# limanling/clip-event

Hardware: AMD Instinct MI355X
Metric: image-text pairs/sec/GPU, ViT-B/32 224px x 77-tok, global-batch contrastive (higher is better)
Workload: dtype bf16; 1 GPU; ViT-B/32 224px x 77-tok, bf16 operands, per-GPU batch 256, K=1, InfoNCE only, full train step (fwd+bwd+clip_grad_norm+Adam), random-init weights; global_batch=256, parallelism=dp1, captions=SOT + U[8,75] random ids + EOT, zero-padded to 77 (SURVEY 8(d) c2), text_rows=live tokens SOT..EOT only: 54.8% of B*77 rows (identical results, see DESIGN.md), fresh_captions_every_step=True, alignment=False, cu_hog=0, nt_pgrid=256, full=False

## Files before the change

### clip_event_amd/csrc/embed.hip

```cpp
#include <limits.h>

#include "common.hpp"
#include "../../include/clip_event_hip.h"

namespace {

__device__ __forceinline__ void im2col_group(const float* __restrict__ img, bf16_t* __restrict__ out_row, int b, int gy,
                                             int gx, int cg, int R, int ps) {
    if (ps % 8 == 0 && R % 4 == 0) {
        const int col = cg * 8;
        u32x4 pk = {0u, 0u, 0u, 0u};
        if (col < 3 * ps * ps) {
            const int c = col / (ps * ps), py = (col / ps) % ps, px = col % ps;
            const float* src = img + (((long)b * 3 + c) * R + gy * ps + py) * R + gx * ps + px;
            const f32x4 lo = __builtin_nontemporal_load(reinterpret_cast<const f32x4*>(src));
            const f32x4 hi = __builtin_nontemporal_load(reinterpret_cast<const f32x4*>(src + 4));
            pk = u32x4{pack_bf2(lo[0], lo[1]), pack_bf2(lo[2], lo[3]), pack_bf2(hi[0], hi[1]), pack_bf2(hi[2], hi[3])};
        }
        *reinterpret_cast<u32x4*>(out_row + cg * 8) = pk;
        return;
    }
    float v[8];
#pragma unroll
    for (int e = 0; e < 8; ++e) {
// ... 365 lines not shown
    }
    if (lane == 0) rows[r] = (int)(r * Ltok + arg);
}

__global__ void copy_rows_kernel(const char* __restrict__ src, long src_stride, const int* __restrict__ src_rows,
                                 char* __restrict__ dst, long dst_stride, const int* __restrict__ dst_rows, int n,
                                 int chunks) {
    const long total = (long)n * chunks;
    for (long idx = blockIdx.x * (long)blockDim.x + threadIdx.x; idx < total; idx += (long)gridDim.x * blockDim.x) {
        const int i = (int)(idx / chunks), c = (int)(idx - (long)i * chunks);
        const long sr = src_rows ? src_rows[i] : i, dr = dst_rows ? dst_rows[i] : i;
        *reinterpret_cast<u32x4*>(dst + dr * dst_stride + c * 16L) =
            *reinterpret_cast<const u32x4*>(src + sr * src_stride + c * 16L);
    }
}

__global__ void scatter_rows_zero_kernel(const char* __restrict__ src, long src_stride, char* __restrict__ dst, long dst_stride,
                                         const int* __restrict__ dst_rows, int n, int M, int chunks) {
    const long total = (long)M * chunks;
    for (long idx = blockIdx.x * (long)blockDim.x + threadIdx.x; idx < total; idx += (long)gridDim.x * blockDim.x) {
        const int r = (int)(idx / chunks), c = (int)(idx - (long)r * chunks);
        int lo = 0, hi = n - 1;
        while (lo < hi) {
            const int mid = (lo + hi) >> 1;
            if (dst_rows[mid] < r) lo = mid + 1;
            else hi = mid;
        }
        u32x4 v = {0u, 0u, 0u, 0u};
        if (dst_rows[lo] == r) v = *reinterpret_cast<const u32x4*>(src + (long)lo * src_stride + c * 16L);
        *reinterpret_cast<u32x4*>(dst + (long)r * dst_stride + c * 16L) = v;
    }
}

int grid_for(long threads, int block = 256, int cap = 8192) {
    long g = (threads + block - 1) / block;
    return (int)(g > cap ? cap : (g < 1 ? 1 : g));
}

}

extern "C" int ce_im2col(const float* image, void* patches, int B, int resolution, int patch, int k_padded,
                         void* stream) {
    CE_CHECK_ARG(B > 0 && patch > 0 && resolution % patch == 0, "ce_im2col: resolution %d not a multiple of patch %d", resolution, patch);
    CE_CHECK_ARG(k_padded % 8 == 0 && k_padded >= 3 * patch * patch, "ce_im2col: k_padded must be a multiple of 8 >= 3*patch^2");
    const int grid = resolution / patch;
    const long threads = (long)B * grid * grid * (k_padded / 8);
    hipLaunchKernelGGL(im2col_kernel, dim3(grid_for(threads)), dim3(256), 0, (hipStream_t)stream, image,
                       (bf16_t*)patches, B, resolution, patch, grid, k_padded);
    CE_LAUNCH_CHECK();
    return 0;
}

extern "C" int ce_vision_assemble(const float* patch_out, const float* cls, const float* pos, float* x0, int B,
                                  int tokens, int D, void* stream) {
    CE_CHECK_ARG(B > 0 && tokens > 1 && D % 4 == 0, "ce_vision_assemble: bad shape");
    hipLaunchKernelGGL(vision_assemble_kernel, dim3(grid_for((long)B * tokens * (D / 4))), dim3(256), 0,
                       (hipStream_t)stream, patch_out, cls, pos, x0, B, tokens, D);
    CE_LAUNCH_CHECK();
    return 0;
}

extern "C" int ce_vision_assemble_bwd(const float* dx0, void* dpatch, int B, int tokens, int D, void* stream) {
    CE_CHECK_ARG(B > 0 && tokens > 1 && D % 4 == 0, "ce_vision_assemble_bwd: bad shape");
    hipLaunchKernelGGL(vision_assemble_bwd_kernel, dim3(grid_for((long)B * (tokens - 1) * (D / 4))), dim3(256), 0,
                       (hipStream_t)stream, dx0, (bf16_t*)dpatch, B, tokens, D);
    CE_LAUNCH_CHECK();
// ... 149 lines not shown
    return 0;
}

extern "C" int ce_scatter_rows_zero(const void* src, long src_stride_bytes, void* dst, long dst_stride_bytes,
                                    const int* dst_rows, int n, int M, int row_bytes, void* stream) {
    CE_CHECK_ARG(n > 0 && M >= n && row_bytes > 0 && row_bytes % 16 == 0 && src_stride_bytes % 16 == 0 && dst_stride_bytes % 16 == 0 &&
                 dst_rows, "ce_scatter_rows_zero: rows must be multiples of 16 bytes, 0 < n <= M");
    const int chunks = row_bytes / 16;
    hipLaunchKernelGGL(scatter_rows_zero_kernel, dim3(grid_for((long)M * chunks)), dim3(256), 0, (hipStream_t)stream,
                       (const char*)src, src_stride_bytes, (char*)dst, dst_stride_bytes, dst_rows, n, M, chunks);
    CE_LAUNCH_CHECK();
    return 0;
}

extern "C" int ce_eot_rows(const int64_t* ids, int* rows, long n, int tokens, void* stream) {
    CE_CHECK_ARG(n > 0 && tokens > 0, "ce_eot_rows: bad shape");
    hipLaunchKernelGGL(eot_rows_kernel, dim3((unsigned)((n + 3) / 4)), dim3(256), 0, (hipStream_t)stream,
                       (const long*)ids, rows, n, tokens);
    CE_LAUNCH_CHECK();
    return 0;
}

extern "C" int ce_copy_rows(const void* src, long src_stride_bytes, const int* src_rows, void* dst,
                            long dst_stride_bytes, const int* dst_rows, int n, int row_bytes, void* stream) {
    CE_CHECK_ARG(n > 0 && row_bytes > 0 && row_bytes % 16 == 0 && src_stride_bytes % 16 == 0 && dst_stride_bytes % 16 == 0,
                 "ce_copy_rows: rows must be multiples of 16 bytes");
    const int chunks = row_bytes / 16;
    hipLaunchKernelGGL(copy_rows_kernel, dim3(grid_for((long)n * chunks)), dim3(256), 0, (hipStream_t)stream,
                       (const char*)src, src_stride_bytes, src_rows, (char*)dst, dst_stride_bytes, dst_rows, n, chunks);
    CE_LAUNCH_CHECK();
    return 0;
}

namespace {
__global__ __launch_bounds__(256) void cu_hog_kernel(unsigned long long ticks, unsigned int* sink, int mode) {
    extern __shared__ unsigned int hog_lds[];
    const unsigned long long t0 = __builtin_amdgcn_s_memrealtime(), c0 = __builtin_amdgcn_s_memtime();
    unsigned int n = 0;
    while (__builtin_amdgcn_s_memrealtime() - t0 < ticks) {
        if (mode == 0) __builtin_amdgcn_s_sleep(32);
        else if (mode == 1) __builtin_amdgcn_s_sleep(127);
        ++n;
    }
    hog_lds[threadIdx.x & 255] = n;
    if (sink && threadIdx.x == 0 && blockIdx.x == 0) {
        const unsigned long long c1 = __builtin_amdgcn_s_memtime(), r1 = __builtin_amdgcn_s_memrealtime();
        reinterpret_cast<unsigned long long*>(sink)[0] = c1 - c0;
        reinterpret_cast<unsigned long long*>(sink)[1] = r1 - t0;
        sink[4] = hog_lds[(threadIdx.x + 1) & 255];
    }
}
}

static unsigned int* g_hog_sink = nullptr;
extern "C" double ce_cu_hog_clock_mhz(void) {
    if (!g_hog_sink) return 0.0;
    unsigned long long h[2] = {0, 0};
    hipDeviceSynchronize();
    hipMemcpy(h, g_hog_sink, sizeof(h), hipMemcpyDeviceToHost);
    return h[1] ? (double)h[0] / (double)h[1] * 100.0 : 0.0;
}

extern "C" int ce_cu_hog(int blocks, float microseconds, void* stream) {
    CE_CHECK_ARG(blocks > 0 && blocks <= 256 && microseconds > 0.f && microseconds <= 1.0e6f, "ce_cu_hog: blocks 1..256, time up to 1 s");
    static bool attr = false;
    if (!attr) {
// ... 16 lines not shown
```

### clip_event_amd/csrc/gemm.hip

```cpp
#include <stdlib.h>

#include <map>
#include <mutex>
#include <type_traits>

#include "common.hpp"
#include "nt_plan.hpp"
#include "tn_plan.hpp"
#include "../../include/clip_event_hip.h"

#ifndef CE_DIAG_TN3
#define CE_DIAG_TN3 0
#endif

namespace {

constexpr int NT_BM = 128, NT_BN = 128, NT_BK = 64;
constexpr int NT_STAGE_BYTES = (NT_BM + NT_BN) * NT_BK * 2;
constexpr int NT_LDS_BYTES = 2 * NT_STAGE_BYTES;

#include "gemm_common.hpp"

template <int EPI>
__global__ __launch_bounds__(256, 2) void gemm_nt_kernel(NTArgs p) {
// ... 1247 lines not shown
#pragma unroll
    for (int nt = 0; nt < 2; ++nt)
#pragma unroll
        for (int kt = 0; kt < 2; ++kt) {
            const int k = ek + kt * 32;
            if (k >= p.Kk) continue;
#pragma unroll
            for (int r = 0; r < 16; ++r) {
                const int n = en + nt * 32 + (r & 3) + 8 * (r >> 2);
                if (n < p.Nn) atomicAdd(p.out + (long)n * p.ldo + k, acc[nt][kt][r]);
            }
        }
}

constexpr int T2_TILE_BYTES = TN_BM * 256;
constexpr int T2_STAGE_BYTES = 2 * T2_TILE_BYTES;
constexpr int T2_LDS_BYTES = 2 * T2_STAGE_BYTES;

__device__ __forceinline__ bf16x8 tr_frag2(const char* p) {
    typedef __attribute__((address_space(3))) s16x4 lds_s16x4;
    s16x4 lo = __builtin_amdgcn_ds_read_tr16_b64_v4i16((lds_s16x4*)(p));
    s16x4 hi = __builtin_amdgcn_ds_read_tr16_b64_v4i16((lds_s16x4*)(p + 4 * 256));
    typedef __attribute__((ext_vector_type(8))) short s16x8;
    s16x8 v = {lo[0], lo[1], lo[2], lo[3], hi[0], hi[1], hi[2], hi[3]};
    return __builtin_bit_cast(bf16x8, v);
}

struct TNGroup {
    int count, splits, m_per_split, M, depth;
    int overwrite = 0;
    int tile_end[CE_TN_MAX_GROUP];
    TNArgs prob[CE_TN_MAX_GROUP];
};

__global__ __launch_bounds__(256, 2) void gemm_tn2_kernel(TNGroup grp) {
    extern __shared__ __attribute__((aligned(16))) char smem[];
    const int tid = threadIdx.x;
    const int lane = tid & 63;
    const int wave = __builtin_amdgcn_readfirstlane(tid >> 6);
    const int wn = wave >> 1, wk = wave & 1;

    const int m_tiles = (grp.M + TN_BM - 1) / TN_BM;
    const int mps = grp.m_per_split / TN_BM;
    const int s_r = lane >> 4;
    const int s_chunk = (lane & 15) ^ (s_r << 2);
    const int g = lane >> 4, li = lane & 15;
    const int t_row = 8 * (g >> 1) + (li >> 2);
    const int t_sw = (li >> 2) << 2;
    const int t_cb = 2 * (g & 1) + ((li & 3) >> 1);
    int offP[2], offQ[2];
#pragma unroll
    for (int t = 0; t < 2; ++t) {
        offP[t] = t_row * 256 + (((wn * 8 + t * 4 + t_cb) ^ t_sw) << 4) + (li & 1) * 8;
        offQ[t] = T2_TILE_BYTES + t_row * 256 + (((wk * 8 + t * 4 + t_cb) ^ t_sw) << 4) + (li & 1) * 8;
    }

    {
        const int lb = xcd_remap(blockIdx.x, gridDim.x);
        int tile = lb / grp.splits;
        const int mt0 = (lb - tile * grp.splits) * mps;
        const int mt1 = min(m_tiles, mt0 + mps);
        if (mt0 >= mt1) return;
        int pi = 0;
        while (pi + 1 < grp.count && tile >= grp.tile_end[pi]) ++pi;
        if (pi > 0) tile -= grp.tile_end[pi - 1];
        const TNArgs& p = grp.prob[pi];
// ... 624 lines not shown

extern "C" int ce_gemm_tn_grouped_ex(int count, const void* const* P, const long* ldp, const void* const* Q,
                                     const long* ldq, int M, const int* Nn, const int* Kk, float* const* out,
                                     const long* ldo, int splits, int overwrite, void* stream) {
    CE_CHECK_ARG(count >= 1 && count <= CE_TN_MAX_GROUP && M > 0, "ce_gemm_tn_grouped: 1..%d problems, M > 0", CE_TN_MAX_GROUP);
    hipStream_t s = (hipStream_t)stream;
    TNGroup g;
    g.count = count;
    g.M = M;
    double flops = 0.0, bytes = 0.0;
    long ldmax = 0;
    for (int i = 0; i < count; ++i) {
        CE_CHECK_ARG(Nn[i] > 0 && Kk[i] > 0, "ce_gemm_tn: empty problem");
        CE_CHECK_ARG(Nn[i] % 8 == 0 && Kk[i] % 8 == 0 && ldp[i] % 8 == 0 && ldq[i] % 8 == 0,
                     "ce_gemm_tn: Nn,Kk,ldp,ldq must be multiples of 8");
        CE_CHECK_ARG(ldp[i] >= Nn[i] && ldq[i] >= Kk[i] && ldo[i] >= Kk[i], "ce_gemm_tn: leading dimension smaller than the row");
        TNArgs& a = g.prob[i];
        a.P = (const bf16_t*)P[i]; a.ldp = ldp[i]; a.Q = (const bf16_t*)Q[i]; a.ldq = ldq[i];
        a.out = out[i]; a.ldo = ldo[i]; a.M = M; a.Nn = Nn[i]; a.Kk = Kk[i];
        flops += 2.0 * M * Nn[i] * Kk[i];
        bytes += 2.0 * ((double)M * Nn[i] + (double)M * Kk[i]) + 8.0 * Nn[i] * Kk[i];
        if (ldp[i] > ldmax) ldmax = ldp[i];
        if (ldq[i] > ldmax) ldmax = ldq[i];
    }
    CE_CHECK_ARG((long)M * ldmax * 2 < (1L << 32), "ce_gemm_tn: operand exceeds 4 GiB");

    const TNPlan p = tn_plan(M, count, Nn, Kk, splits, overwrite != 0, tn_process_knobs());
    g.splits = p.splits; g.m_per_split = p.m_per_split; g.depth = p.depth; g.overwrite = p.kernel_overwrites;
    for (int i = 0; i < CE_TN_MAX_GROUP; ++i) g.tile_end[i] = p.tile_end[i];
    for (int i = 0; i < count; ++i) {
        TNArgs& a = g.prob[i];
        a.tiles_n = p.tiles_n[i]; a.tiles_k = p.tiles_k[i]; a.splits = p.splits; a.m_per_split = p.m_per_split;
    }
    if (p.zero_fill_first)
        for (int i = 0; i < count; ++i)
            if (hipMemset2DAsync(out[i], (size_t)ldo[i] * 4, 0, (size_t)Kk[i] * 4, (size_t)Nn[i], s) != hipSuccess) {
                ce_set_error("ce_gemm_tn_grouped: zero-fill of output %d failed", i);
                return -5;
            }

    constexpr auto key = [](int form, int rows) { return 64 * form + rows; };
#define CE_TN_CASE(FORM, ROWS, ...)                                                      \
    case key(FORM, ROWS): {                                                              \
        CeProfScope prof(p.prof_class, flops, bytes, s);                                 \
        launch_kernel<__VA_ARGS__>(p.workgroups, p.block, p.lds_bytes, g, s);            \
    } break
    switch (key(p.form, p.rows)) {
        case key(TN_V1, 64):
            for (int i = 0; i < count; ++i) {
                const TNArgs& a = g.prob[i];
                CeProfScope prof(p.prof_class, 2.0 * M * a.Nn * a.Kk, 0.0, s);
                launch_kernel<gemm_tn_kernel>(a.tiles_n * a.tiles_k * a.splits, p.block, p.lds_bytes, a, s);
            }
            break;
        CE_TN_CASE(TN_V2, 64, gemm_tn2_kernel);
        CE_TN_CASE(TN_V3, 32, gemm_tn3_kernel<32, 4>);
        CE_TN_CASE(TN_V3, 48, gemm_tn3_kernel<48, 3>);
        CE_TN_CASE(TN_V3LW, 48, gemm_tn3lw_kernel<48, 3>);
        CE_TN_CASE(TN_V3LW, 32, gemm_tn3lw_kernel<32, 4>);
        default: CE_CHECK_ARG(false, "ce_gemm_tn_grouped: no kernel of form %d with %d-row stages", (int)p.form, p.rows);
    }
#undef CE_TN_CASE
    CE_LAUNCH_CHECK();
    return 0;
}

extern "C" int ce_gemm_tn_plan(int count, const int* Nn, const int* Kk, int M, int splits, int overwrite, const ce_tn_knobs* knobs,
// ... 29 lines not shown
```

### clip_event_amd/csrc/layernorm.hip

```cpp
#include <stdlib.h>

#include "common.hpp"
#include "../../include/clip_event_hip.h"

namespace {

__device__ __forceinline__ __amdgpu_buffer_rsrc_t row_rsrc(const void* base, long row, long ld, int esz, int D) {
    return make_rsrc(reinterpret_cast<const char*>(base) + row * ld * esz, (uint32_t)(D * esz));
}
#ifndef CE_LN_NT
#define CE_LN_NT 0
#endif
template <int T> struct Raw4 { typedef u32x2 type; };
template <> struct Raw4<CE_T_F32> { typedef f32x4 type; };
template <int T, int AUX = 0>
__device__ __forceinline__ typename Raw4<T>::type ld4_row(__amdgpu_buffer_rsrc_t r, int c) {
    if constexpr (T == CE_T_F32) return __builtin_bit_cast(f32x4, __builtin_amdgcn_raw_buffer_load_b128(r, c * 4, 0, AUX));
    else return __builtin_amdgcn_raw_buffer_load_b64(r, c * 2, 0, AUX);
}
template <int T>
__device__ __forceinline__ f32x4 cvt4(typename Raw4<T>::type raw) {
    if constexpr (T == CE_T_F32) return raw;
    else if constexpr (T == CE_T_F16) return f16x4_to_f32(raw);
    else return f32x4{bf_lo(raw[0]), bf_hi(raw[0]), bf_lo(raw[1]), bf_hi(raw[1])};
// ... 241 lines not shown
        }
        __syncthreads();
        for (int c = threadIdx.x; c < D; c += 64 * NW) {
            float t = 0.f;
#pragma unroll
            for (int wv = 0; wv < NW; ++wv) t += red[wv * D + c];
            strip[pass * D + c] = t;
        }
    }
    __syncthreads();
    const int total = P * D;
    if (partial) {
        float* pp = partial + (size_t)blockIdx.x * 3 * D;
        for (int j = threadIdx.x; j < total; j += 64 * NW) pp[j] = strip[j];
        return;
    }
    const int start = (int)((blockIdx.x * 64u) % (unsigned)total);
    for (int j = threadIdx.x; j < total; j += 64 * NW) {
        int e = j + start;
        if (e >= total) e -= total;
        const int pass = e >= 2 * D ? 2 : (e >= D ? 1 : 0);
        float* dstp = pass == 0 ? dw : (pass == 1 ? db : dxsum);
#ifndef CE_DIAG_LN_NO_ATOMICS
        atomicAdd(dstp + (e - pass * D), strip[e]);
#else
        if (strip[e] == 123.456f) dstp[e - pass * D] = strip[e];
#endif
    }
}

struct LnFoldJobs {
    ce_ln_fold_job job[CE_LN_FOLD_MAX];
};
__global__ __launch_bounds__(256) void ln_fold_kernel(LnFoldJobs jobs) {
    const ce_ln_fold_job& jb = jobs.job[blockIdx.y];
    const int D = jb.D, P = jb.dxsum ? 3 : 2;
    const int j = blockIdx.x * 256 + threadIdx.x;
    if (j >= P * D) return;
    float t = 0.f;
    const float* pp = jb.partials + j;
#pragma unroll 8
    for (int b = 0; b < jb.blocks; ++b) t += pp[(size_t)b * 3 * D];
    const int pass = j / D, c = j - pass * D;
    float* dst = pass == 0 ? jb.dw : (pass == 1 ? jb.db : jb.dxsum);
    dst[c] += t;
}

}

#define LN_DISPATCH(D, CALL)                                     \
    do {                                                         \
        if ((D) <= 256) { CALL(1); }                             \
        else if ((D) <= 512) { CALL(2); }                        \
        else if ((D) <= 768) { CALL(3); }                        \
        else if ((D) <= 1024) { CALL(4); }                       \
        else { CALL(8); }                                        \
    } while (0)

extern "C" int ce_layernorm_fwd_t(const void* x, int x_type, long ldx, const int* rows, const float* w, const float* b,
                                  void* y, int y_type, long ldy, float* mean, float* rstd, int M, int D, float eps,
                                  void* stream) {
    return ce_layernorm_fwd_q8(x, x_type, ldx, rows, w, b, y, y_type, ldy, mean, rstd, M, D, eps, nullptr, 0, nullptr, stream);
}

extern "C" int ce_layernorm_fwd_q8(const void* x, int x_type, long ldx, const int* rows, const float* w, const float* b,
                                   void* y, int y_type, long ldy, float* mean, float* rstd, int M, int D, float eps,
                                   void* q8v, long ldq, float* qscale, void* stream) {
    uint8_t* q8 = reinterpret_cast<uint8_t*>(q8v);
    CE_CHECK_ARG(!q8 || (y_type == CE_T_BF16 && qscale && ldq >= D && ldq % 4 == 0), "ce_layernorm_fwd_q8: the e4m3 copy needs a bf16 output, scales and ldq >= D");
    CE_CHECK_ARG(M > 0 && D > 0 && D % 4 == 0 && D <= 2048, "ce_layernorm_fwd: need 0<D<=2048, D%%4==0 (D=%d M=%d)", D, M);
    CE_CHECK_ARG(ldx % 4 == 0 && ldy % 4 == 0, "ce_layernorm_fwd: leading dimensions must be multiples of 4");
    static const int rpw_env = getenv("CE_LN_FWD_RPW") ? atoi(getenv("CE_LN_FWD_RPW")) : 0;
    const int rpw = D > 1024 ? 1 : (rpw_env == 2 ? 2 : 1);
    dim3 grid(ce_div_up(M, 4 * rpw)), block(256);
    hipStream_t s = (hipStream_t)stream;
    unsigned int* sat = ce_sat_counters();
    CeProfScope prof(CE_PROF_LN_FWD, 8.0 * M * D, (double)(ce_type_bytes(x_type) + ce_type_bytes(y_type)) * M * D, s);
    const int combo = x_type * 4 + y_type;
// ... 45 lines not shown

extern "C" int ce_layernorm_bwd_q8(const void* dy, int dy_type, long lddy, const void* x, int x_type, long ldx,
                                   const int* rows, const float* mean, const float* rstd, const float* w,
                                   const void* dx_in, int dxin_type, void* dx_out, int dx_type, long lddx, void* dxb,
                                   long lddxb, float* dw, float* db, float* dxsum, const float* gscale, int M, int D,
                                   void* q8v, long ldq, float* qscale, void* stream) {
    return ln_bwd_launch(dy, dy_type, lddy, x, x_type, ldx, rows, mean, rstd, w, dx_in, dxin_type, dx_out, dx_type, lddx, dxb, lddxb, dw, db,
                         dxsum, gscale, M, D, q8v, ldq, qscale, nullptr, stream);
}

extern "C" int ce_layernorm_bwd_partials(const void* dy, int dy_type, long lddy, const void* x, int x_type, long ldx,
                                         const int* rows, const float* mean, const float* rstd, const float* w,
                                         const void* dx_in, int dxin_type, void* dx_out, int dx_type, long lddx, void* dxb,
                                         long lddxb, int want_dxsum, const float* gscale, int M, int D, void* q8v, long ldq,
                                         float* qscale, float* partials, void* stream) {
    CE_CHECK_ARG(partials, "ce_layernorm_bwd_partials: null partials buffer");
    float* tag = partials;
    return ln_bwd_launch(dy, dy_type, lddy, x, x_type, ldx, rows, mean, rstd, w, dx_in, dxin_type, dx_out, dx_type, lddx, dxb, lddxb, tag, tag,
                         want_dxsum ? tag : nullptr, gscale, M, D, q8v, ldq, qscale, partials, stream);
}

extern "C" int ce_layernorm_fold(const ce_ln_fold_job* jobs, int njobs, void* stream) {
    CE_CHECK_ARG(jobs && njobs > 0, "ce_layernorm_fold: no jobs");
    for (int base = 0; base < njobs; base += CE_LN_FOLD_MAX) {
        LnFoldJobs pack;
        const int n = njobs - base < CE_LN_FOLD_MAX ? njobs - base : CE_LN_FOLD_MAX;
        int maxd = 0;
        for (int i = 0; i < n; ++i) {
            pack.job[i] = jobs[base + i];
            CE_CHECK_ARG(pack.job[i].partials && pack.job[i].dw && pack.job[i].db && pack.job[i].blocks > 0 && pack.job[i].D > 0,
                         "ce_layernorm_fold: job %d incomplete", base + i);
            if (pack.job[i].D > maxd) maxd = pack.job[i].D;
        }
        hipLaunchKernelGGL(ln_fold_kernel, dim3(ce_div_up(3 * maxd, 256), n), dim3(256), 0, (hipStream_t)stream, pack);
    }
    CE_LAUNCH_CHECK();
    return 0;
}

static int ln_bwd_launch(const void* dy, int dy_type, long lddy, const void* x, int x_type, long ldx,
                         const int* rows, const float* mean, const float* rstd, const float* w,
                         const void* dx_in, int dxin_type, void* dx_out, int dx_type, long lddx, void* dxb,
                         long lddxb, float* dw, float* db, float* dxsum, const float* gscale, int M, int D,
                         void* q8v, long ldq, float* qscale, float* partial, void* stream) {
    uint8_t* q8 = reinterpret_cast<uint8_t*>(q8v);
    CE_CHECK_ARG(!q8 || (dxb && qscale && ldq >= D && ldq % 4 == 0), "ce_layernorm_bwd_q8: the e4m3 copy is a copy of dxb (needs dxb, scales, ldq >= D)");
    CE_CHECK_ARG(M > 0 && D > 0 && D % 4 == 0 && D <= 2048, "ce_layernorm_bwd: need 0<D<=2048, D%%4==0 (D=%d M=%d)", D, M);
    CE_CHECK_ARG(lddy % 4 == 0 && ldx % 4 == 0 && lddx % 4 == 0 && lddxb % 4 == 0, "ce_layernorm_bwd: leading dimensions must be multiples of 4");
    if (!dx_in) dxin_type = CE_T_F32;
    CE_CHECK_ARG(gscale || (dy_type != CE_T_F16 && dxin_type != CE_T_F16 && dx_type != CE_T_F16),
                 "ce_layernorm_bwd: an fp16 gradient operand needs the device scale (ce_grad_scale)");
    const int nw = D <= 512 ? 16 : (D <= 1024 ? 8 : 4);
    const int blocks = ln_bwd_blocks(M, D);
    dim3 grid(blocks), block(64 * nw);
    const size_t lds = (size_t)(nw + 3) * D * sizeof(float);
    hipStream_t s = (hipStream_t)stream;
    unsigned int* sat = ce_sat_counters();
    CeProfScope prof(CE_PROF_LN_BWD, 16.0 * M * D,
                     (double)(ce_type_bytes(dy_type) + ce_type_bytes(x_type) + (dx_in ? ce_type_bytes(dxin_type) : 0) +
                              ce_type_bytes(dx_type) + (dxb ? 2 : 0)) * M * D, s);
    const int combo = ((dy_type * 4 + x_type) * 4 + dxin_type) * 4 + dx_type;
#define LNB(DYT, XT, DIT, DOT) (((DYT * 4 + XT) * 4 + DIT) * 4 + DOT)
#define LAUNCH(IT, DYT, XT, DIT, DOT)                                                                                         \
    hipLaunchKernelGGL((ln_bwd_kernel<IT, (IT <= 2 ? 16 : (IT <= 4 ? 8 : 4)), DYT, XT, DIT, DOT, true>), grid, block, lds, s, dy, lddy, \
                       x, ldx, rows, mean, rstd, w, dx_in, dx_out, lddx, (bf16_t*)dxb, lddxb, dw, db, dxsum, gscale, M, D, q8, ldq, qscale, partial, sat)
#define CALL(IT)                                                                                                              \
    switch (combo) {                                                                                                          \
// ... 27 lines not shown
```

### clip_event_amd/csrc/tower.cpp

```cpp
#include <hip/hip_runtime.h>
#include <stdlib.h>

#include <map>
#include <mutex>

#include "common.hpp"
#include "tn_plan.hpp"
#include "../../include/clip_event_hip.h"

namespace {

constexpr int WG_MAX_BLOCKS = TN_GROUP_MAX_BLOCKS;
constexpr int WG_SETS = WG_MAX_BLOCKS + 1;
constexpr int LNP_RING = 8;

struct Carver {
    char* base;
    size_t off = 0;
    explicit Carver(void* b) : base(reinterpret_cast<char*>(b)) {}
    template <typename T>
    T* take(size_t n) {
        off = (off + 255) & ~size_t(255);
        T* p = base ? reinterpret_cast<T*>(base + off) : nullptr;
        off += n * sizeof(T);
// ... 119 lines not shown
           long ldo2, const void* aux, long ldaux, void* stream) {
    if (use8 && W8 && S8 && K % 128 == 0 && K <= 4096) {
        if (q8_of != A || lda != K) TRY(ce_quant_rows_fp8(A, lda, L.q8, K, L.q8s, M, K, stream));
        q8_of = nullptr;
        return ce_gemm_nt_fp8(L.q8, K, L.q8s, W8, K, S8, M, N, K, epi, bias, resid, ldr, out, ldo, out2, ldo2, aux, ldaux,
                              stream);
    }
    return ce_gemm_nt(A, lda, W, K, M, N, K, epi, bias, resid, ldr, out, ldo, out2, ldo2, aux, ldaux, stream);
}

int forward_run(const ce_tower_desc* d, int batch, int rows, const int* cu_seqlens, const void* x0, Layout& L, void* x_out,
                const int* sel_rows, bool infer, void* stream) {
    const int M = rows, w = d->width;
    const bool f8 = (d->fp8 & 1) != 0;
    const int ST = d->stream16 ? CE_T_F16 : CE_T_F32;
    const int EPI_RESID = d->stream16 ? CE_EPI_BIAS_RESID_F16 : CE_EPI_BIAS_RESID_F32;
    const int EPI_FC = infer ? CE_EPI_BIAS_QGELU_BF16 : CE_EPI_BIAS_GELU;
    const long esz = d->stream16 ? 2 : 4;
    const void* x = x0;
    const void* q8_of = nullptr;
    const bool lnq = f8 && w % 128 == 0 && w <= 4096;
    for (int l = 0; l < d->layers; ++l) {
        const ce_block_params& p = d->blocks[l];
        BlockStash& s = L.blk[l];
        void* xo = (l + 1 < d->layers) ? s.x_out : x_out;
        TRY(ce_layernorm_fwd_q8(x, ST, w, nullptr, p.ln1_w, p.ln1_b, s.h1, CE_T_BF16, w, s.mean1, s.rstd1, M, w, 1e-5f,
                                lnq ? L.q8 : nullptr, w, L.q8s, stream));
        if (lnq) q8_of = s.h1;
        TRY(linear(f8, L, q8_of, s.h1, w, p.w_qkv, p.w8_qkv, p.s8_qkv, M, 3 * w, w, CE_EPI_BIAS_BF16, p.b_qkv, nullptr, 0, s.qkv, 3 * w, nullptr, 0,
                       nullptr, 0, stream));
        TRY(ce_attention_fwd(s.qkv, 3 * w, s.o, w, s.lse, cu_seqlens, batch, d->tokens, d->heads, d->causal, stream));
        if (sel_rows && l + 1 == d->layers) {
            const int Bn = batch;
            TRY(ce_copy_rows(s.o, w * 2L, sel_rows, L.os, w * 2L, nullptr, Bn, w * 2, stream));
            TRY(ce_copy_rows(x, w * esz, sel_rows, L.xs_in, w * esz, nullptr, Bn, (int)(w * esz), stream));
            TRY(linear(f8, L, q8_of, L.os, w, p.w_out, p.w8_out, p.s8_out, Bn, w, w, EPI_RESID, p.b_out, L.xs_in, w, L.xs_mid, w, nullptr,
                           0, nullptr, 0, stream));
            TRY(ce_layernorm_fwd_t(L.xs_mid, ST, w, nullptr, p.ln2_w, p.ln2_b, L.h2s, CE_T_BF16, w, L.means, L.rstds, Bn, w, 1e-5f, stream));
            TRY(linear(f8, L, q8_of, L.h2s, w, p.w_fc, p.w8_fc, p.s8_fc, Bn, 4 * w, w, EPI_FC, p.b_fc, nullptr, 0, infer ? L.gs : L.as, 4 * w,
                           infer ? nullptr : L.gs, infer ? 0 : 4 * w, nullptr, 0, stream));
            TRY(linear(f8, L, q8_of, L.gs, 4 * w, p.w_proj, p.w8_proj, p.s8_proj, Bn, w, 4 * w, EPI_RESID, p.b_proj, L.xs_mid, w, x_out, w,
                           nullptr, 0, nullptr, 0, stream));
            break;
        }
        TRY(linear(f8, L, q8_of, s.o, w, p.w_out, p.w8_out, p.s8_out, M, w, w, EPI_RESID, p.b_out, x, w, s.x_mid, w, nullptr, 0, nullptr,
                       0, stream));
        TRY(ce_layernorm_fwd_q8(s.x_mid, ST, w, nullptr, p.ln2_w, p.ln2_b, s.h2, CE_T_BF16, w, s.mean2, s.rstd2, M, w, 1e-5f,
                                lnq ? L.q8 : nullptr, w, L.q8s, stream));
        if (lnq) q8_of = s.h2;
        TRY(linear(f8, L, q8_of, s.h2, w, p.w_fc, p.w8_fc, p.s8_fc, M, 4 * w, w, EPI_FC, p.b_fc, nullptr, 0, infer ? s.g : s.a, 4 * w,
                       infer ? nullptr : s.g, infer ? 0 : 4 * w, nullptr, 0, stream));
        TRY(linear(f8, L, q8_of, s.g, 4 * w, p.w_proj, p.w8_proj, p.s8_proj, M, w, 4 * w, EPI_RESID, p.b_proj, s.x_mid, w, xo, w,
                       nullptr, 0, nullptr, 0, stream));
        x = xo;
    }
    return 0;
}

}

extern "C" size_t ce_tower_workspace_bytes(const ce_tower_desc* d, int batch) {
    if (check_desc(d, batch) != 0) return 0;
    Layout L;
    carve(d, batch, (size_t)batch * d->tokens, nullptr, L);
    return L.bytes;
}

extern "C" int ce_tower_forward(const ce_tower_desc* d, int batch, int rows, const int* cu_seqlens, const void* x0,
// ... 78 lines not shown
        for (int i = 0; i < groups; ++i) {
            l -= sizes[i];
            cut_after[l + 1] = true;
        }
    };
    struct Pending {
        const void* P[CE_TN_MAX_GROUP]; long ldp[CE_TN_MAX_GROUP];
        const void* Q[CE_TN_MAX_GROUP]; long ldq[CE_TN_MAX_GROUP];
        int Nn[CE_TN_MAX_GROUP], Kk[CE_TN_MAX_GROUP];
        float* out[CE_TN_MAX_GROUP]; long ldo[CE_TN_MAX_GROUP];
        int count = 0, blocks = 0;
    } pend;
    auto queue = [&](const void* P, long ldp, const void* Q, long ldq, int Nn, int Kk, float* out, long ldo) {
        const int i = pend.count++;
        pend.P[i] = P; pend.ldp[i] = ldp; pend.Q[i] = Q; pend.ldq[i] = ldq;
        pend.Nn[i] = Nn; pend.Kk[i] = Kk; pend.out[i] = out; pend.ldo[i] = ldo;
    };
    auto flush = [&]() -> int {
        if (pend.count == 0) return 0;
        const int rc = ce_gemm_tn_grouped_ex(pend.count, pend.P, pend.ldp, pend.Q, pend.ldq, M, pend.Nn, pend.Kk, pend.out,
                                             pend.ldo, 0, d->wgrad_overwrite, stream);
        pend.count = 0;
        pend.blocks = 0;
        return rc;
    };
    int top = layer_hi;
    if (layer_hi < last) {
    } else if (sel_rows) {
        CE_CHECK_ARG(dx_sel, "ce_tower_backward: pruned mode needs dx_sel");
        const int l = top, Bn = batch, q = l % WG_SETS;
        const ce_block_params& p = d->blocks[l];
        BlockStash& s = L.blk[l];
        const void* x_in = (l == 0) ? x0 : L.blk[l - 1].x_out;
        TRY(ce_cast_bf16(dx_sel, L.dxbs, (long)Bn * w, stream));
        TRY(linear(b8, L, q8_of, L.dxbs, w, p.wt_proj, p.wt8_proj, p.st8_proj, Bn, 4 * w, w, CE_EPI_GELUGRAD_BF16, nullptr, nullptr, 0, L.das, 4 * w, nullptr,
                       0, L.as, 4 * w, stream));
        TRY(ce_colsum_bf16(L.dxbs, w, p.g_b_proj, Bn, w, stream));
        TRY(linear(b8, L, q8_of, L.das, 4 * w, p.wt_fc, p.wt8_fc, p.st8_fc, Bn, w, 4 * w, CE_EPI_BF16, nullptr, nullptr, 0, L.dhs, w, nullptr, 0,
                       nullptr, 0, stream));
        TRY(ce_colsum_bf16(L.das, 4 * w, p.g_b_fc, Bn, 4 * w, stream));
        TRY(ce_layernorm_bwd_t(L.dhs, CE_T_BF16, w, L.xs_mid, ST, w, nullptr, L.means, L.rstds, p.ln2_w, dx_sel, CE_T_F32, L.dxs_mid,
                               ST, w, L.dxb2s, w, p.g_ln2_w, p.g_ln2_b, p.g_b_out, GS, Bn, w, stream));
        TRY(linear(b8, L, q8_of, L.dxb2s, w, p.wt_out, p.wt8_out, p.st8_out, Bn, w, w, CE_EPI_BF16, nullptr, nullptr, 0, L.dos, w, nullptr, 0, nullptr, 0,
                       stream));
        TRY(ce_scatter_rows_zero(L.dos, w * 2L, L.d_o, w * 2L, sel_rows, Bn, M, w * 2, stream));
        TRY(ce_attention_bwd(s.qkv, 3 * w, s.o, w, L.d_o, w, s.lse, L.dqkv[q], 3 * w, p.g_b_qkv, cu_seqlens, batch, d->tokens, d->heads,
                             d->causal, stream));
        {
            const void* P[3] = {L.dxbs, L.das, L.dxb2s};
            const long ldp[3] = {w, 4L * w, w};
            const void* Q[3] = {L.gs, L.h2s, L.os};
            const long ldq[3] = {4L * w, w, w};
            const int Nn[3] = {w, 4 * w, w};
            const int Kk[3] = {4 * w, w, w};
            float* out[3] = {p.g_w_proj, p.g_w_fc, p.g_w_out};
            const long ldo[3] = {4L * w, w, w};
            TRY(ce_gemm_tn_grouped_ex(3, P, ldp, Q, ldq, Bn, Nn, Kk, out, ldo, 0, d->wgrad_overwrite, stream));
        }
        queue(L.dqkv[q], 3L * w, s.h1, w, 3 * w, w, p.g_w_qkv, w);
        TRY(linear(b8, L, q8_of, L.dqkv[q], 3 * w, p.wt_qkv, p.wt8_qkv, p.st8_qkv, M, w, 3 * w, CE_EPI_BF16, nullptr, nullptr, 0, L.dh, w, nullptr, 0,
                       nullptr, 0, stream));
        TRY(ce_scatter_rows_zero(L.dxs_mid, w * esz, dx, w * esz, sel_rows, Bn, M, (int)(w * esz), stream));
        TRY(ce_layernorm_bwd_t(L.dh, CE_T_BF16, w, x_in, ST, w, nullptr, s.mean1, s.rstd1, p.ln1_w, dx, ST, dx, ST, w,
                               L.dxb[(l + WG_SETS - 1) % WG_SETS], w, p.g_ln1_w, p.g_ln1_b,
                               (l > 0) ? d->blocks[l - 1].g_b_proj : nullptr, GS, M, w, stream));
        top = l - 1;
    } else {
        if (d->stream16) TRY(ce_cast_scaled(dx, ST, L.dxb[top % WG_SETS], CE_T_BF16, GS, 1, (long)M * w, stream));
        else TRY(ce_cast_bf16(reinterpret_cast<const float*>(dx), L.dxb[top % WG_SETS], (long)M * w, stream));
    }
    plan_cuts(top, layer_lo, pend.count > 0 ? 3 * tn_problem_tiles(M, w, w) : 0);
    for (int l = top; l >= layer_lo; --l) {
        const ce_block_params& p = d->blocks[l];
        BlockStash& s = L.blk[l];
        const int q = l % WG_SETS;
        bf16_t *dxb_a = L.dxb[q], *dxb_b = L.dxb2[q], *da = L.da[q], *dqkv = L.dqkv[q];
        const void* x_in = (l == 0) ? x0 : L.blk[l - 1].x_out;
        TRY(linear(b8, L, q8_of, dxb_a, w, p.wt_proj, p.wt8_proj, p.st8_proj, M, 4 * w, w, CE_EPI_GELUGRAD_BF16, nullptr, nullptr, 0, da, 4 * w, p.g_b_fc,
                       4 * w, s.a, 4 * w, stream));
        if (l == last) TRY(ce_colsum_bf16(dxb_a, w, p.g_b_proj, M, w, stream));
        TRY(linear(b8, L, q8_of, da, 4 * w, p.wt_fc, p.wt8_fc, p.st8_fc, M, w, 4 * w, CE_EPI_BF16, nullptr, nullptr, 0, L.dh, w, nullptr, 0,
                       nullptr, 0, stream));
        TRY(ln_bwd(L.dh, s.x_mid, s.mean2, s.rstd2, p.ln2_w, dxb_b, p.g_ln2_w, p.g_ln2_b, p.g_b_out, lnq ? L.q8 : nullptr, L.lnp[l % LNP_RING][1]));
        if (lnq) q8_of = dxb_b;
        TRY(linear(b8, L, q8_of, dxb_b, w, p.wt_out, p.wt8_out, p.st8_out, M, w, w, CE_EPI_BF16, nullptr, nullptr, 0, L.d_o, w, nullptr, 0, nullptr, 0,
                       stream));
        TRY(ce_attention_bwd(s.qkv, 3 * w, s.o, w, L.d_o, w, s.lse, dqkv, 3 * w, p.g_b_qkv, cu_seqlens, batch, d->tokens, d->heads,
                             d->causal, stream));
        queue(dxb_a, w, s.g, 4L * w, w, 4 * w, p.g_w_proj, 4L * w);
        queue(da, 4L * w, s.h2, w, 4 * w, w, p.g_w_fc, w);
        queue(dxb_b, w, s.o, w, w, w, p.g_w_out, w);
        queue(dqkv, 3L * w, s.h1, w, 3 * w, w, p.g_w_qkv, w);
        ++pend.blocks;
        if (cut_after[l] || pend.count + 4 > CE_TN_MAX_GROUP) TRY(flush());
        TRY(linear(b8, L, q8_of, dqkv, 3 * w, p.wt_qkv, p.wt8_qkv, p.st8_qkv, M, w, 3 * w, CE_EPI_BF16, nullptr, nullptr, 0, L.dh, w, nullptr, 0,
// ... 16 lines not shown
```

### include/clip_event_hip.h

```cpp
#ifndef CLIP_EVENT_HIP_H
#define CLIP_EVENT_HIP_H

#include <stddef.h>
#include <stdint.h>

#ifdef __cplusplus
extern "C" {
#endif

const char* ce_last_error(void);
int ce_version(void);

enum {
    CE_EPI_BF16 = 0,
    CE_EPI_F32 = 1,
    CE_EPI_BIAS_BF16 = 2,
    CE_EPI_BIAS_F32 = 3,
    CE_EPI_BIAS_RESID_F32 = 4,
    CE_EPI_BIAS_GELU = 5,
    CE_EPI_GELUGRAD_BF16 = 6,
    CE_EPI_BIAS_RESID_F16 = 7,
    CE_EPI_BIAS_QGELU_BF16 = 8
};

// ... 79 lines not shown

int ce_im2col(const float* image, void* patches, int B, int resolution, int patch, int k_padded, void* stream);
int ce_vision_assemble(const float* patch_out, const float* cls, const float* pos, float* x0, int B, int tokens,
                       int D, void* stream);
int ce_vision_assemble_bwd(const float* dx0, void* dpatch, int B, int tokens, int D, void* stream);
int ce_patch_keep(long seed, long draw, long sample0, int B, int N, int keep, int* keep_idx, int* inv, void* stream);
int ce_im2col_rows(const float* image, const int* keep_idx, void* patches, int B, int keep, int resolution, int patch,
                   int k_padded, void* stream);
int ce_vision_assemble_rows(const float* patch_out, const int* keep_idx, const float* cls, const float* pos, float* x0,
                            int B, int N, int keep, int D, void* stream);
int ce_pos_embed_bwd_rows(const float* dx0, const int* inv, float* dpos, int B, int N, int keep, int D, void* stream);
int ce_token_embed(const int64_t* ids, const int* src_rows, const float* table, const float* pos, float* x0, long rows,
                   int tokens, int D, int vocab, void* stream);
int ce_token_embed_t(const int64_t* ids, const int* src_rows, const float* table, const float* pos, void* x0, int x0_type,
                     long rows, int tokens, int D, int vocab, void* stream);
int ce_token_embed_bwd(const int64_t* ids, const int* src_rows, const float* dx0, float* dtable, long rows, int D,
                       int vocab, void* stream);
int ce_pos_embed_bwd_packed(const float* dx0, const int* cu_seqlens, float* dpos, int n, int tokens, int D,
                            void* stream);
int ce_batch_reduce(const float* x, float* out, int B, long slab, long n, int accumulate, void* stream);
int ce_colsum_bf16(const void* x, long ld, float* out, int M, int N, void* stream);
int ce_cast_transpose(const float* w, void* w16, long ld16, void* w16t, long ld16t, int R, int C, void* stream);
int ce_cast_bf16(const float* x, void* y, long n, void* stream);
int ce_cast_t(const void* x, int src_type, void* y, int dst_type, float mul, long n, void* stream);
int ce_cast_scaled(const void* x, int src_type, void* y, int dst_type, const float* scale, int divide, long n, void* stream);
#define CE_GRAD_SCALE_SCRATCH 256
int ce_grad_scale(const float* x, long n, float target, float* scratch, float* scale, void* stream);
int ce_stream16_set_counters(unsigned int* device_counters);
int ce_add_cols(const float* src, long lds, float* dst, long ldd, int rows, int cols, void* stream);
int ce_copy_rows(const void* src, long src_stride_bytes, const int* src_rows, void* dst, long dst_stride_bytes,
                 const int* dst_rows, int n, int row_bytes, void* stream);
int ce_scatter_rows_zero(const void* src, long src_stride_bytes, void* dst, long dst_stride_bytes, const int* dst_rows, int n,
                         int M, int row_bytes, void* stream);
int ce_eot_rows(const int64_t* ids, int* rows, long n, int tokens, void* stream);

typedef struct {
    const unsigned char* src;
    long pitch;
    int x0, y0, w, h;
    int ow, oh;
    int left, top;
    int row0, rows;
    long tmp_off;
} ce_preproc_desc;
size_t ce_preprocess_table_bytes(int n_out, int n_px, int kmax);
int ce_preprocess(const ce_preproc_desc* descs_device, int n_out, int n_px, int kmax, int max_rows, void* table,
                  void* tmp, float* out, const float* mean, const float* std, void* stream);

enum { CE_AUG_BRIGHTNESS = 0, CE_AUG_CONTRAST = 1, CE_AUG_SATURATION = 2, CE_AUG_HUE = 3 };
typedef struct {
    int flip;
    int grey;
    int n_ops;
    int op[4];
    float factor[4];
} ce_augment_desc;
size_t ce_augment_workspace_bytes(int n_out, int n_px, int kmax, long tmp_bytes);
int ce_augment(const ce_preproc_desc* descs_device, const ce_augment_desc* augs_device, const ce_augment_desc* augs_host,
               int n_out, int n_px, int kmax, int max_rows, void* workspace, float* out, const float* mean, const float* std,
               void* stream);

int ce_l2norm_fwd(const float* f, long ldf, float* y, long ldy, float* inv_norm, int n, int E, void* stream);
int ce_l2norm_bwd(const float* dy, long lddy, const float* y, long ldy, const float* inv_norm, float* df, long lddf,
                  int n, int E, int accumulate, void* stream);
int ce_sgemm(const float* A, long sam, long sak, const float* B, long sbk, long sbn, float* C, long ldc, int M,
             int N, int K, const float* alpha_ptr, float alpha, int alpha_exp, float beta, void* stream);
// ... 244 lines not shown
```

Measured before the change: 20690 pairs/s (whole job).

## Fuse small row-gather, scatter, cast+colsum and TN zero-fill kernels; widen LN fold reduction

Merges paired row gather/scatter launches in the last-layer selected-row path into single dual-buffer kernels, and fuses the bf16 cast of dx with its bias column sum. Replaces per-output hipMemset2D zero-fills in grouped TN GEMM with one zero kernel, and splits the LayerNorm fold reduction across 8 row groups per column block with a shared-memory reduction. The goal is fewer tiny launches and better parallelism in small reduction kernels. The colsum now sums bf16-rounded values computed in-kernel, and it uses atomics, so the accumulation order can vary from run to run.

```diff
diff --git a/clip_event_amd/csrc/embed.hip b/clip_event_amd/csrc/embed.hip
--- a/clip_event_amd/csrc/embed.hip
+++ b/clip_event_amd/csrc/embed.hip
@@ -421,6 +421,90 @@
     }
 }
 
+__global__ void gather_rows2_kernel(const char* __restrict__ src_a, long sa_stride, char* __restrict__ dst_a, long da_stride, int ca,
+                                    const char* __restrict__ src_b, long sb_stride, char* __restrict__ dst_b, long db_stride, int cb,
+                                    const int* __restrict__ rows, int n) {
+    const int chunks = ca + cb;
+    const long total = (long)n * chunks;
+    for (long idx = blockIdx.x * (long)blockDim.x + threadIdx.x; idx < total; idx += (long)gridDim.x * blockDim.x) {
+        const int i = (int)(idx / chunks), c = (int)(idx - (long)i * chunks);
+        const long sr = rows ? rows[i] : i;
+        if (c < ca)
+            *reinterpret_cast<u32x4*>(dst_a + i * da_stride + c * 16L) = *reinterpret_cast<const u32x4*>(src_a + sr * sa_stride + c * 16L);
+        else
+            *reinterpret_cast<u32x4*>(dst_b + i * db_stride + (c - ca) * 16L) =
+                *reinterpret_cast<const u32x4*>(src_b + sr * sb_stride + (c - ca) * 16L);
+    }
+}
+
+__global__ void scatter_rows_zero2_kernel(const char* __restrict__ src_a, long sa_stride, char* __restrict__ dst_a, long da_stride, int ca,
+                                          const char* __restrict__ src_b, long sb_stride, char* __restrict__ dst_b, long db_stride, int cb,
+                                          const int* __restrict__ dst_rows, int n, int M) {
+    const int chunks = ca + cb;
+    const long total = (long)M * chunks;
+    for (long idx = blockIdx.x * (long)blockDim.x + threadIdx.x; idx < total; idx += (long)gridDim.x * blockDim.x) {
+        const int r = (int)(idx / chunks), c = (int)(idx - (long)r * chunks);
+        int lo = 0, hi = n - 1;
+        while (lo < hi) {
+            const int mid = (lo + hi) >> 1;
+            if (dst_rows[mid] < r) lo = mid + 1;
+            else hi = mid;
+        }
+        const bool hit = dst_rows[lo] == r;
+        u32x4 v = {0u, 0u, 0u, 0u};
+        if (c < ca) {
+            if (hit) v = *reinterpret_cast<const u32x4*>(src_a + (long)lo * sa_stride + c * 16L);
+            *reinterpret_cast<u32x4*>(dst_a + (long)r * da_stride + c * 16L) = v;
+        } else {
+            if (hit) v = *reinterpret_cast<const u32x4*>(src_b + (long)lo * sb_stride + (c - ca) * 16L);
+            *reinterpret_cast<u32x4*>(dst_b + (long)r * db_stride + (c - ca) * 16L) = v;
+        }
+    }
+}
+
+__global__ __launch_bounds__(256) void cast_colsum_bf16_kernel(const float* __restrict__ x, long ldx, bf16_t* __restrict__ y, long ldy,
+                                                               float* __restrict__ out, int M, int N) {
+    __shared__ float red[8][257];
+    const int cg = threadIdx.x & 31, rg = threadIdx.x >> 5;
+    const int c = blockIdx.x * 256 + cg * 8;
+    float acc[8] = {0.f, 0.f, 0.f, 0.f, 0.f, 0.f, 0.f, 0.f};
+    if (c < N) {
+        const int r0 = blockIdx.y * 64 + rg;
+#pragma unroll
+        for (int h = 0; h < 2; ++h) {
+            u32x4 v[4];
+#pragma unroll
+            for (int u = 0; u < 4; ++u) {
+                const int r = r0 + (h * 4 + u) * 8;
+                v[u] = u32x4{0u, 0u, 0u, 0u};
+                if (r < M) {
+                    const f32x4 lo = *reinterpret_cast<const f32x4*>(x + (long)r * ldx + c);
+                    const f32x4 hi = *reinterpret_cast<const f32x4*>(x + (long)r * ldx + c + 4);
+                    v[u] = u32x4{pack_bf2(lo[0], lo[1]), pack_bf2(lo[2], lo[3]), pack_bf2(hi[0], hi[1]), pack_bf2(hi[2], hi[3])};
+                    *reinterpret_cast<u32x4*>(y + (long)r * ldy + c) = v[u];
+                }
+            }
+#pragma unroll
+            for (int u = 0; u < 4; ++u)
+#pragma unroll
+                for (int e = 0; e < 4; ++e) {
+                    acc[2 * e] += bf_lo(v[u][e]);
+                    acc[2 * e + 1] += bf_hi(v[u][e]);
+                }
+        }
+    }
+#pragma unroll
+    for (int e = 0; e < 8; ++e) red[rg][cg * 8 + e] = acc[e];
+    __syncthreads();
+    const int col = blockIdx.x * 256 + threadIdx.x;
+    if (col < N) {
+        float t = 0.f;
+#pragma unroll
+        for (int g = 0; g < 8; ++g) t += red[g][threadIdx.x];
+        atomicAdd(out + col, t);
+    }
+}
+
 int grid_for(long threads, int block = 256, int cap = 8192) {
     long g = (threads + block - 1) / block;
     return (int)(g > cap ? cap : (g < 1 ? 1 : g));
@@ -636,6 +720,47 @@
     return 0;
 }
 
+extern "C" int ce_gather_rows2(const void* src_a, long src_a_stride_bytes, void* dst_a, long dst_a_stride_bytes, int row_bytes_a,
+                               const void* src_b, long src_b_stride_bytes, void* dst_b, long dst_b_stride_bytes, int row_bytes_b,
+                               const int* src_rows, int n, void* stream) {
+    CE_CHECK_ARG(src_a && dst_a && src_b && dst_b && n > 0, "ce_gather_rows2: null buffer or no rows");
+    CE_CHECK_ARG(row_bytes_a > 0 && row_bytes_b > 0 && row_bytes_a % 16 == 0 && row_bytes_b % 16 == 0 && src_a_stride_bytes % 16 == 0 &&
+                 dst_a_stride_bytes % 16 == 0 && src_b_stride_bytes % 16 == 0 && dst_b_stride_bytes % 16 == 0,
+                 "ce_gather_rows2: rows must be multiples of 16 bytes");
+    const int ca = row_bytes_a / 16, cb = row_bytes_b / 16;
+    hipLaunchKernelGGL(gather_rows2_kernel, dim3(grid_for((long)n * (ca + cb))), dim3(256), 0, (hipStream_t)stream, (const char*)src_a,
+                       src_a_stride_bytes, (char*)dst_a, dst_a_stride_bytes, ca, (const char*)src_b, src_b_stride_bytes, (char*)dst_b,
+                       dst_b_stride_bytes, cb, src_rows, n);
+    CE_LAUNCH_CHECK();
+    return 0;
+}
+
+extern "C" int ce_scatter_rows_zero2(const void* src_a, long src_a_stride_bytes, void* dst_a, long dst_a_stride_bytes, int row_bytes_a,
+                                     const void* src_b, long src_b_stride_bytes, void* dst_b, long dst_b_stride_bytes, int row_bytes_b,
+                                     const int* dst_rows, int n, int M, void* stream) {
+    CE_CHECK_ARG(src_a && dst_a && src_b && dst_b && dst_rows && n > 0 && M >= n, "ce_scatter_rows_zero2: null buffer, or not 0 < n <= M");
+    CE_CHECK_ARG(row_bytes_a > 0 && row_bytes_b > 0 && row_bytes_a % 16 == 0 && row_bytes_b % 16 == 0 && src_a_stride_bytes % 16 == 0 &&
+                 dst_a_stride_bytes % 16 == 0 && src_b_stride_bytes % 16 == 0 && dst_b_stride_bytes % 16 == 0,
+                 "ce_scatter_rows_zero2: rows must be multiples of 16 bytes");
+    const int ca = row_bytes_a / 16, cb = row_bytes_b / 16;
+    hipLaunchKernelGGL(scatter_rows_zero2_kernel, dim3(grid_for((long)M * (ca + cb))), dim3(256), 0, (hipStream_t)stream,
+                       (const char*)src_a, src_a_stride_bytes, (char*)dst_a, dst_a_stride_bytes, ca, (const char*)src_b,
+                       src_b_stride_bytes, (char*)dst_b, dst_b_stride_bytes, cb, dst_rows, n, M);
+    CE_LAUNCH_CHECK();
+    return 0;
+}
+
+extern "C" int ce_cast_colsum_bf16(const float* x, long ldx, void* y, long ldy, float* out, int M, int N, void* stream) {
+    CE_CHECK_ARG(x && y && out && M > 0 && N > 0, "ce_cast_colsum_bf16: null buffer or empty matrix");
+    CE_CHECK_ARG(N % 8 == 0 && ldx % 4 == 0 && ldy % 8 == 0 && ldx >= N && ldy >= N,
+                 "ce_cast_colsum_bf16: N and ldy must be multiples of 8, ldx of 4, and no smaller than N");
+    CeProfScope prof(CE_PROF_COLSUM, (double)M * N, 6.0 * M * N, (hipStream_t)stream);
+    hipLaunchKernelGGL(cast_colsum_bf16_kernel, dim3(ce_div_up(N, 256), ce_div_up(M, 64)), dim3(256), 0, (hipStream_t)stream, x, ldx,
+                       (bf16_t*)y, ldy, out, M, N);
+    CE_LAUNCH_CHECK();
+    return 0;
+}
+
 namespace {
 __global__ __launch_bounds__(256) void cu_hog_kernel(unsigned long long ticks, unsigned int* sink, int mode) {
     extern __shared__ unsigned int hog_lds[];
diff --git a/clip_event_amd/csrc/gemm.hip b/clip_event_amd/csrc/gemm.hip
--- a/clip_event_amd/csrc/gemm.hip
+++ b/clip_event_amd/csrc/gemm.hip
@@ -1303,6 +1303,17 @@
     int tile_end[CE_TN_MAX_GROUP];
     TNArgs prob[CE_TN_MAX_GROUP];
 };
+
+__global__ __launch_bounds__(256) void tn_zero_outputs_kernel(TNGroup grp) {
+    const TNArgs& p = grp.prob[blockIdx.y];
+    const int chunks = p.Kk / 4;
+    const long total = (long)p.Nn * chunks;
+    for (long idx = blockIdx.x * (long)blockDim.x + threadIdx.x; idx < total; idx += (long)gridDim.x * blockDim.x) {
+        const long n = idx / chunks;
+        const int c = (int)(idx - n * chunks);
+        *reinterpret_cast<f32x4*>(p.out + n * p.ldo + c * 4) = f32x4{0.f, 0.f, 0.f, 0.f};
+    }
+}
 
 __global__ __launch_bounds__(256, 2) void gemm_tn2_kernel(TNGroup grp) {
     extern __shared__ __attribute__((aligned(16))) char smem[];
@@ -1993,7 +2004,16 @@
         TNArgs& a = g.prob[i];
         a.tiles_n = p.tiles_n[i]; a.tiles_k = p.tiles_k[i]; a.splits = p.splits; a.m_per_split = p.m_per_split;
     }
-    if (p.zero_fill_first)
+    bool zero_aligned = count > 1;
+    long zero_chunks = 0;
+    for (int i = 0; i < count; ++i) {
+        zero_aligned = zero_aligned && reinterpret_cast<uintptr_t>(out[i]) % 16 == 0 && ldo[i] % 4 == 0;
+        if ((long)Nn[i] * (Kk[i] / 4) > zero_chunks) zero_chunks = (long)Nn[i] * (Kk[i] / 4);
+    }
+    if (p.zero_fill_first && zero_aligned) {
+        const long wgs = (zero_chunks + 255) / 256;
+        hipLaunchKernelGGL(tn_zero_outputs_kernel, dim3((unsigned)(wgs > 2048 ? 2048 : wgs), count), dim3(256), 0, s, g);
+    } else if (p.zero_fill_first)
         for (int i = 0; i < count; ++i)
             if (hipMemset2DAsync(out[i], (size_t)ldo[i] * 4, 0, (size_t)Kk[i] * 4, (size_t)Nn[i], s) != hipSuccess) {
                 ce_set_error("ce_gemm_tn_grouped: zero-fill of output %d failed", i);
diff --git a/clip_event_amd/csrc/layernorm.hip b/clip_event_amd/csrc/layernorm.hip
--- a/clip_event_amd/csrc/layernorm.hip
+++ b/clip_event_amd/csrc/layernorm.hip
@@ -297,18 +297,29 @@
 struct LnFoldJobs {
     ce_ln_fold_job job[CE_LN_FOLD_MAX];
 };
-__global__ __launch_bounds__(256) void ln_fold_kernel(LnFoldJobs jobs) {
+constexpr int LN_FOLD_COLS = 32, LN_FOLD_RG = 8;
+__global__ __launch_bounds__(LN_FOLD_COLS * LN_FOLD_RG) void ln_fold_kernel(LnFoldJobs jobs) {
+    __shared__ float red[LN_FOLD_RG][LN_FOLD_COLS + 1];
     const ce_ln_fold_job& jb = jobs.job[blockIdx.y];
     const int D = jb.D, P = jb.dxsum ? 3 : 2;
-    const int j = blockIdx.x * 256 + threadIdx.x;
-    if (j >= P * D) return;
+    if (blockIdx.x * LN_FOLD_COLS >= P * D) return;
+    const int cl = threadIdx.x % LN_FOLD_COLS, rg = threadIdx.x / LN_FOLD_COLS;
+    const int j = blockIdx.x * LN_FOLD_COLS + cl;
     float t = 0.f;
-    const float* pp = jb.partials + j;
+    if (j < P * D) {
+        const float* pp = jb.partials + j;
 #pragma unroll 8
-    for (int b = 0; b < jb.blocks; ++b) t += pp[(size_t)b * 3 * D];
+        for (int b = rg; b < jb.blocks; b += LN_FOLD_RG) t += pp[(size_t)b * 3 * D];
+    }
+    red[rg][cl] = t;
+    __syncthreads();
+    if (rg != 0 || j >= P * D) return;
+    float s = red[0][cl];
+#pragma unroll
+    for (int g = 1; g < LN_FOLD_RG; ++g) s += red[g][cl];
     const int pass = j / D, c = j - pass * D;
     float* dst = pass == 0 ? jb.dw : (pass == 1 ? jb.db : jb.dxsum);
-    dst[c] += t;
+    dst[c] += s;
 }
 
 }
@@ -420,7 +431,8 @@
                          "ce_layernorm_fold: job %d incomplete", base + i);
             if (pack.job[i].D > maxd) maxd = pack.job[i].D;
         }
-        hipLaunchKernelGGL(ln_fold_kernel, dim3(ce_div_up(3 * maxd, 256), n), dim3(256), 0, (hipStream_t)stream, pack);
+        hipLaunchKernelGGL(ln_fold_kernel, dim3(ce_div_up(3 * maxd, LN_FOLD_COLS), n), dim3(LN_FOLD_COLS * LN_FOLD_RG), 0,
+                           (hipStream_t)stream, pack);
     }
     CE_LAUNCH_CHECK();
     return 0;
diff --git a/clip_event_amd/csrc/tower.cpp b/clip_event_amd/csrc/tower.cpp
--- a/clip_event_amd/csrc/tower.cpp
+++ b/clip_event_amd/csrc/tower.cpp
@@ -175,8 +175,7 @@
         TRY(ce_attention_fwd(s.qkv, 3 * w, s.o, w, s.lse, cu_seqlens, batch, d->tokens, d->heads, d->causal, stream));
         if (sel_rows && l + 1 == d->layers) {
             const int Bn = batch;
-            TRY(ce_copy_rows(s.o, w * 2L, sel_rows, L.os, w * 2L, nullptr, Bn, w * 2, stream));
-            TRY(ce_copy_rows(x, w * esz, sel_rows, L.xs_in, w * esz, nullptr, Bn, (int)(w * esz), stream));
+            TRY(ce_gather_rows2(s.o, w * 2L, L.os, w * 2L, w * 2, x, w * esz, L.xs_in, w * esz, (int)(w * esz), sel_rows, Bn, stream));
             TRY(linear(f8, L, q8_of, L.os, w, p.w_out, p.w8_out, p.s8_out, Bn, w, w, EPI_RESID, p.b_out, L.xs_in, w, L.xs_mid, w, nullptr,
                            0, nullptr, 0, stream));
             TRY(ce_layernorm_fwd_t(L.xs_mid, ST, w, nullptr, p.ln2_w, p.ln2_b, L.h2s, CE_T_BF16, w, L.means, L.rstds, Bn, w, 1e-5f, stream));
@@ -321,10 +320,9 @@
         const ce_block_params& p = d->blocks[l];
         BlockStash& s = L.blk[l];
         const void* x_in = (l == 0) ? x0 : L.blk[l - 1].x_out;
-        TRY(ce_cast_bf16(dx_sel, L.dxbs, (long)Bn * w, stream));
+        TRY(ce_cast_colsum_bf16(dx_sel, w, L.dxbs, w, p.g_b_proj, Bn, w, stream));
         TRY(linear(b8, L, q8_of, L.dxbs, w, p.wt_proj, p.wt8_proj, p.st8_proj, Bn, 4 * w, w, CE_EPI_GELUGRAD_BF16, nullptr, nullptr, 0, L.das, 4 * w, nullptr,
                        0, L.as, 4 * w, stream));
-        TRY(ce_colsum_bf16(L.dxbs, w, p.g_b_proj, Bn, w, stream));
         TRY(linear(b8, L, q8_of, L.das, 4 * w, p.wt_fc, p.wt8_fc, p.st8_fc, Bn, w, 4 * w, CE_EPI_BF16, nullptr, nullptr, 0, L.dhs, w, nullptr, 0,
                        nullptr, 0, stream));
         TRY(ce_colsum_bf16(L.das, 4 * w, p.g_b_fc, Bn, 4 * w, stream));
@@ -332,7 +330,7 @@
                                ST, w, L.dxb2s, w, p.g_ln2_w, p.g_ln2_b, p.g_b_out, GS, Bn, w, stream));
         TRY(linear(b8, L, q8_of, L.dxb2s, w, p.wt_out, p.wt8_out, p.st8_out, Bn, w, w, CE_EPI_BF16, nullptr, nullptr, 0, L.dos, w, nullptr, 0, nullptr, 0,
                        stream));
-        TRY(ce_scatter_rows_zero(L.dos, w * 2L, L.d_o, w * 2L, sel_rows, Bn, M, w * 2, stream));
+        TRY(ce_scatter_rows_zero2(L.dos, w * 2L, L.d_o, w * 2L, w * 2, L.dxs_mid, w * esz, dx, w * esz, (int)(w * esz), sel_rows, Bn, M, stream));
         TRY(ce_attention_bwd(s.qkv, 3 * w, s.o, w, L.d_o, w, s.lse, L.dqkv[q], 3 * w, p.g_b_qkv, cu_seqlens, batch, d->tokens, d->heads,
                              d->causal, stream));
         {
@@ -349,7 +347,6 @@
         queue(L.dqkv[q], 3L * w, s.h1, w, 3 * w, w, p.g_w_qkv, w);
         TRY(linear(b8, L, q8_of, L.dqkv[q], 3 * w, p.wt_qkv, p.wt8_qkv, p.st8_qkv, M, w, 3 * w, CE_EPI_BF16, nullptr, nullptr, 0, L.dh, w, nullptr, 0,
                        nullptr, 0, stream));
-        TRY(ce_scatter_rows_zero(L.dxs_mid, w * esz, dx, w * esz, sel_rows, Bn, M, (int)(w * esz), stream));
         TRY(ce_layernorm_bwd_t(L.dh, CE_T_BF16, w, x_in, ST, w, nullptr, s.mean1, s.rstd1, p.ln1_w, dx, ST, dx, ST, w,
                                L.dxb[(l + WG_SETS - 1) % WG_SETS], w, p.g_ln1_w, p.g_ln1_b,
                                (l > 0) ? d->blocks[l - 1].g_b_proj : nullptr, GS, M, w, stream));
diff --git a/include/clip_event_hip.h b/include/clip_event_hip.h
--- a/include/clip_event_hip.h
+++ b/include/clip_event_hip.h
@@ -135,6 +135,13 @@
                  const int* dst_rows, int n, int row_bytes, void* stream);
 int ce_scatter_rows_zero(const void* src, long src_stride_bytes, void* dst, long dst_stride_bytes, const int* dst_rows, int n,
                          int M, int row_bytes, void* stream);
+int ce_gather_rows2(const void* src_a, long src_a_stride_bytes, void* dst_a, long dst_a_stride_bytes, int row_bytes_a,
+                    const void* src_b, long src_b_stride_bytes, void* dst_b, long dst_b_stride_bytes, int row_bytes_b,
+                    const int* src_rows, int n, void* stream);
+int ce_scatter_rows_zero2(const void* src_a, long src_a_stride_bytes, void* dst_a, long dst_a_stride_bytes, int row_bytes_a,
+                          const void* src_b, long src_b_stride_bytes, void* dst_b, long dst_b_stride_bytes, int row_bytes_b,
+                          const int* dst_rows, int n, int M, void* stream);
+int ce_cast_colsum_bf16(const float* x, long ldx, void* y, long ldy, float* out, int M, int N, void* stream);
 int ce_eot_rows(const int64_t* ids, int* rows, long n, int tokens, void* stream);
 
 typedef struct {
```

Measured after the change: 20640 pairs/s (whole job). No clear change (-0.3%).
